# eezkni/UEGAN

Measured on AMD Instinct MI355X. Metric: train imgs/sec @512px bs=16 on 1/2/4/8 MI355X; infer ms/img, higher is better.
Workload: dtype bf16; 1 GPU; FiveK-shaped 512x512 batch=16/GPU, full G/D/VGG train step (trainer.py:77-119), conv_dim=32, seeded stand-in VGG19; global_batch=16, parallelism=dp1, pool_size=50, collective=none (1 rank), passes=batched (fused.py)

## Files before the change

### include/uegan_hip.h

```cpp
#ifndef UEGAN_HIP_H_
#define UEGAN_HIP_H_

#include <stddef.h>
#include <stdint.h>

#ifdef __cplusplus
extern "C" {
#endif

#define UEGAN_VERSION 105

enum { UEGAN_OK = 0, UEGAN_E_INVALID = -1, UEGAN_E_HIP = -2, UEGAN_E_UNSUPPORTED = -3 };
enum { UEGAN_F32 = 0, UEGAN_BF16 = 1 };
enum { UEGAN_PAD_ZERO = 0, UEGAN_PAD_REFLECT = 1 };
enum { UEGAN_ACT_NONE = 0, UEGAN_ACT_LRELU = 1, UEGAN_ACT_RELU = 2, UEGAN_ACT_TANH = 3,
       UEGAN_ACT_SIGMOID = 4,
       UEGAN_ACT_SWISH = 5, UEGAN_ACT_SELU = 6 };
enum { UEGAN_IMPL_AUTO = 0, UEGAN_IMPL_MFMA = 1, UEGAN_IMPL_DIRECT = 2, UEGAN_IMPL_MFMA_REGSTAGE = 3, UEGAN_IMPL_MFMA_GENERIC = 4 };

typedef void* uegan_stream_t;

int uegan_version(void);
const char* uegan_last_error(void);
int uegan_set_conv_impl(int impl);
enum {
  UEGAN_TUNE_SMALL_GRID = 0,
  UEGAN_TUNE_FOLD_MAX = 1,
  UEGAN_TUNE_HEADS_NO_CG = 2,
  UEGAN_TUNE_WIDE_MIN_GRID = 3,
  UEGAN_TUNE_TALL_MIN_GRID = 4,
  UEGAN_TUNE_TALL_RPW = 5,
  UEGAN_TUNE_TALL_REFLECT = 6,
  UEGAN_TUNE_FLAT_S2 = 7,
  UEGAN_TUNE_TOEP_HEADS = 8,
  UEGAN_TUNE_HEADS_MFMA = 9,
  UEGAN_TUNE_FWD_STATS = 10,
  UEGAN_TUNE_WGRAD_XCD = 11,
  UEGAN_TUNE_COUNT = 12
};
int uegan_set_tuning(int knob, int value, int* previous);
int uegan_selftest_mfma(void* scratch_4096_floats, uegan_stream_t stream);

typedef struct {
  char name[96];
  int64_t launches;
  double total_ms;
  double total_flops;
  double total_bytes;
} uegan_profile_entry;
int uegan_profile_begin(int max_records);
int uegan_profile_end(uegan_profile_entry* out, int max_entries, int* n_entries);

typedef struct {
// ... 71 lines not shown
int uegan_conv2d_fwd_pool_part(const uegan_conv_desc* d, const void* x1, const void* x2, const void* w_ohwi, const float* bias,
                               const float* scale, void* y, void* y_pool, int n_full, uegan_stream_t stream);
int uegan_conv2d_fwd_pool_idx(const uegan_conv_desc* d, const void* x1, const void* x2, const void* w_ohwi, const float* bias,
                              const float* scale, void* y, void* y_pool, void* idx, int n_full, int n_idx, uegan_stream_t stream);
int uegan_conv2d_dgrad(const uegan_conv_desc* d, const void* dz, const void* w_ihwo, const float* scale, void* dx1,
                       void* dx2, uegan_stream_t stream);
size_t uegan_conv2d_dgrad_workspace_bytes(const uegan_conv_desc* d);
int uegan_conv2d_dgrad_ws(const uegan_conv_desc* d, const void* dz, const void* w_ihwo, const float* scale, void* dx1,
                          void* dx2, void* workspace, size_t workspace_bytes, uegan_stream_t stream);
int uegan_conv2d_dgrad_padded(const uegan_conv_desc* d, const void* dz, const void* w_ihwo, const void* w_ohwi, const float* scale,
                              void* workspace, size_t workspace_bytes, int* pad_out, uegan_stream_t stream);
size_t uegan_conv2d_dgrad_padded_bytes(const uegan_conv_desc* d);

int uegan_conv2d_dgrad_act(const uegan_conv_desc* d, const void* dz, const void* w_ihwo, const float* scale, void* dx1,
                           void* workspace, size_t workspace_bytes, int in_act, const void* x_act, uegan_stream_t stream);
size_t uegan_conv2d_wgrad_workspace_bytes(const uegan_conv_desc* d);
int uegan_conv2d_wgrad(const uegan_conv_desc* d, const void* x1, const void* x2, const void* dz, const float* scale,
                       float* dw_oihw, float* dbias, void* workspace, size_t workspace_bytes, uegan_stream_t stream);
int uegan_conv2d_wgrad_acc(const uegan_conv_desc* d, const void* x1, const void* x2, const void* dz, const float* scale,
                           float* dw_oihw, float* dbias, void* workspace, size_t workspace_bytes, int accumulate,
                           uegan_stream_t stream);
int uegan_act_bwd(int dtype, int act, const void* g, const void* a, void* dz, int64_t n, uegan_stream_t stream);
int uegan_act_bwd2(int dtype, int act, const void* g, const void* g2, const void* a, void* dz, int64_t n, uegan_stream_t stream);
int uegan_act_bwd3(int dtype, int act, const void* g, const void* g2, const void* g3, const void* a, void* dz, int64_t n,
                   uegan_stream_t stream);

int uegan_nchw_to_nhwc(int dtype, const float* x_nchw, void* y_nhwc, int B, int C, int Cp, int H, int W, const float* a,
                       const float* b, uegan_stream_t stream);
int uegan_nhwc_to_nchw(int dtype, const void* x_nhwc, float* y_nchw, int B, int C, int Cp, int H, int W, const float* a,
                       uegan_stream_t stream);
// ... 144 lines not shown
```

### uegan_amd/_lib.py

```python
import ctypes as C
import os

_HERE = os.path.dirname(os.path.abspath(__file__))
LIB_PATH = os.path.join(_HERE, "libuegan_hip.so")
LIB_PATH_F16 = os.path.join(_HERE, "libuegan_hip_f16.so")

_lib = None
_lib_f16 = None
_use_f16 = False
_emulated = False

c_int, c_i64, c_f32, c_vp, c_sz = C.c_int, C.c_int64, C.c_float, C.c_void_p, C.c_size_t


class ConvDesc(C.Structure):
    _fields_ = [(n, C.c_int32) for n in ("dtype", "B", "H", "W", "C1", "C2", "Ho", "Wo", "Cout", "KH", "KW", "stride", "pad",
                                          "pad_mode", "act", "Cin_w", "Cout_w", "Cin_total", "scale_group")]


class ProfileEntry(C.Structure):
    _fields_ = [("name", C.c_char * 96), ("launches", c_i64), ("total_ms", C.c_double), ("total_flops", C.c_double),
                ("total_bytes", C.c_double)]


# ... 35 lines not shown
    "uegan_conv2d_fwd_ex": (c_int, [C.POINTER(ConvDesc), C.POINTER(ConvEx), c_vp, c_vp, c_vp, c_vp, c_vp, c_vp, C.POINTER(c_int), c_vp]),
    "uegan_nchw_to_nhwc_pair": (c_int, [c_int, c_vp, c_vp, c_int, c_int, c_int, c_int, c_int, C.POINTER(c_f32), C.POINTER(c_f32), c_vp]),
    "uegan_instnorm_apply_pair": (c_int, [c_int, c_vp, c_vp, c_vp, c_vp, c_vp, c_vp, c_int, c_int, c_int, c_vp]),
    "uegan_conv2d_fwd": (c_int, [C.POINTER(ConvDesc), c_vp, c_vp, c_vp, c_vp, c_vp, c_vp, c_vp]),
    "uegan_conv2d_fwd_splitk_workspace_bytes": (c_sz, [C.POINTER(ConvDesc)]),
    "uegan_conv2d_fwd_splitk": (c_int, [C.POINTER(ConvDesc), c_vp, c_vp, c_vp, c_vp, c_vp, c_vp, c_vp, c_sz, c_vp]),
    "uegan_conv2d_fwd_pool": (c_int, [C.POINTER(ConvDesc), c_vp, c_vp, c_vp, c_vp, c_vp, c_vp, c_vp, c_vp]),
    "uegan_conv2d_fwd_pool_part": (c_int, [C.POINTER(ConvDesc), c_vp, c_vp, c_vp, c_vp, c_vp, c_vp, c_vp, c_int, c_vp]),
    "uegan_conv2d_fwd_pool_idx": (c_int, [C.POINTER(ConvDesc), c_vp, c_vp, c_vp, c_vp, c_vp, c_vp, c_vp, c_vp, c_int, c_int, c_vp]),
    "uegan_maxpool2x2_fwd_idx": (c_int, [c_int, c_vp, c_vp, c_vp, c_int, c_int, c_int, c_int, c_vp]),
    "uegan_maxpool2x2_bwd_idx": (c_int, [c_int, c_int, c_vp, c_vp, c_vp, c_vp, c_int, c_int, c_int, c_int, c_vp]),
    "uegan_conv2d_dgrad": (c_int, [C.POINTER(ConvDesc), c_vp, c_vp, c_vp, c_vp, c_vp, c_vp]),
    "uegan_conv2d_dgrad_workspace_bytes": (c_sz, [C.POINTER(ConvDesc)]),
    "uegan_conv2d_dgrad_ws": (c_int, [C.POINTER(ConvDesc), c_vp, c_vp, c_vp, c_vp, c_vp, c_vp, c_sz, c_vp]),
    "uegan_conv2d_dgrad_act": (c_int, [C.POINTER(ConvDesc), c_vp, c_vp, c_vp, c_vp, c_vp, c_sz, c_int, c_vp, c_vp]),
    "uegan_conv2d_fwd_stats_workspace_bytes": (c_sz, [C.POINTER(ConvDesc)]),
    "uegan_conv2d_fwd_stats": (c_int, [C.POINTER(ConvDesc), c_vp, c_vp, c_vp, c_vp, c_vp, c_vp, c_vp, c_vp, c_f32, c_vp, c_sz, C.POINTER(c_int), c_vp]),
    "uegan_instnorm_apply": (c_int, [c_int, c_vp, c_vp, c_vp, c_vp, c_int, c_int, c_int, c_vp]),
    "uegan_conv2d_dgrad_padded": (c_int, [C.POINTER(ConvDesc), c_vp, c_vp, c_vp, c_vp, c_vp, c_sz, C.POINTER(c_int), c_vp]),
    "uegan_conv2d_dgrad_padded_bytes": (c_sz, [C.POINTER(ConvDesc)]),
    "uegan_conv2d_wgrad_workspace_bytes": (c_sz, [C.POINTER(ConvDesc)]),
    "uegan_conv2d_wgrad": (c_int, [C.POINTER(ConvDesc), c_vp, c_vp, c_vp, c_vp, c_vp, c_vp, c_vp, c_sz, c_vp]),
    "uegan_conv2d_wgrad_acc": (c_int, [C.POINTER(ConvDesc), c_vp, c_vp, c_vp, c_vp, c_vp, c_vp, c_vp, c_sz, c_int, c_vp]),
    "uegan_act_bwd": (c_int, [c_int, c_int, c_vp, c_vp, c_vp, c_i64, c_vp]),
    "uegan_act_bwd2": (c_int, [c_int, c_int, c_vp, c_vp, c_vp, c_vp, c_i64, c_vp]),
    "uegan_act_bwd3": (c_int, [c_int, c_int, c_vp, c_vp, c_vp, c_vp, c_vp, c_i64, c_vp]),
    "uegan_nchw_to_nhwc": (c_int, [c_int, c_vp, c_vp, c_int, c_int, c_int, c_int, c_int, C.POINTER(c_f32), C.POINTER(c_f32), c_vp]),
    "uegan_nhwc_to_nchw": (c_int, [c_int, c_vp, c_vp, c_int, c_int, c_int, c_int, c_int, C.POINTER(c_f32), c_vp]),
    "uegan_residual_clamp_fwd": (c_int, [c_int, c_vp, c_vp, c_vp, c_int, c_int, c_int, c_int, c_int, c_vp]),
    "uegan_residual_clamp_bwd": (c_int, [c_int, c_vp, c_vp, c_vp, c_vp, c_vp, c_int, c_int, c_int, c_int, c_int, c_vp]),
# ... 141 lines not shown
```

### uegan_amd/csrc/common.h

```cpp
#pragma once
#include <hip/hip_runtime.h>
#include <stdint.h>
#include <stddef.h>

#include "../../include/uegan_hip.h"

#ifdef UEGAN_TOOLS_BUILD
#define UEGAN_ABL_BITS(x) (x)
#else
#define UEGAN_ABL_BITS(x) 0
#endif

namespace uegan {

extern int g_tuning[UEGAN_TUNE_COUNT];
extern int g_abl_stream, g_abl_wide;


typedef uint16_t bf16_t;

typedef float f32x4 __attribute__((ext_vector_type(4)));
typedef short s16x8 __attribute__((ext_vector_type(8)));
typedef uint32_t u32x4 __attribute__((ext_vector_type(4)));
typedef uint32_t u32x2 __attribute__((ext_vector_type(2)));
// ... 141 lines not shown
    default: return apply_act_ext(v, act);
  }
}
__device__ __forceinline__ float act_grad_of_pre(float v, int act) {
  switch (act) {
    case UEGAN_ACT_LRELU: return v > 0.f ? 1.f : 0.2f;
    case UEGAN_ACT_RELU: return v > 0.f ? 1.f : 0.f;
    case UEGAN_ACT_TANH: { const float t = tanhf(v); return 1.f - t * t; }
    case UEGAN_ACT_SIGMOID: { const float sg = 1.f / (1.f + expf(-v)); return sg * (1.f - sg); }
    case UEGAN_ACT_SWISH: { const float sg = 1.f / (1.f + expf(-v)); return sg * (1.f + v * (1.f - sg)); }
    case UEGAN_ACT_SELU: return v > 0.f ? UEGAN_SELU_SCALE : (UEGAN_SELU_SCALE * UEGAN_SELU_ALPHA) * expf(v);
    default: return 1.f;
  }
}

__host__ __device__ __forceinline__ int reflect_idx(int i, int n) {
  i = i < 0 ? -i : i;
  return i >= n ? 2 * (n - 1) - i : i;
}

__device__ __forceinline__ float wave_sum(float v) {
#pragma unroll
  for (int o = 32; o > 0; o >>= 1) v += __shfl_xor(v, o, 64);
  return v;
}

__device__ __forceinline__ float block_sum(float v, float* red) {
  v = wave_sum(v);
  const int lane = threadIdx.x & 63, w = threadIdx.x >> 6;
  __syncthreads();
// ... 35 lines not shown
```

### uegan_amd/csrc/conv.hip

```cpp
#include "conv_core.h"

#include <type_traits>

namespace uegan {

static int g_conv_impl = UEGAN_IMPL_AUTO;
int g_tuning[UEGAN_TUNE_COUNT] = {256, -1, 0, 192, 192, 0, 1, 1, 1, 1, 1, 1};
int g_abl_stream = 0, g_abl_wide = 0;
#ifdef UEGAN_TOOLS_BUILD
extern "C" int uegan_tools_set_ablation(int stream_wgrad_bits, int wide_variant) {
  g_abl_stream = stream_wgrad_bits;
  g_abl_wide = wide_variant;
  return UEGAN_OK;
}
#endif

bool g_prof_on = false;
std::vector<ProfRecord> g_prof_records;
std::vector<std::pair<hipEvent_t, hipEvent_t>> g_prof_pool;
size_t g_prof_used = 0;

int conv_patch_bf16_a(ConvArgs& a, hipStream_t s, int ks);
int conv_patch_bf16_b(ConvArgs& a, hipStream_t s, int ks);
int conv_patch_f32_a(ConvArgs& a, hipStream_t s, int ks);
// ... 1709 lines not shown
    g.B = d->B; g.IH = d->Ho; g.IW = d->Wo; g.C1 = d->Cout; g.C2 = 0; g.C = d->Cout;
    g.OH = d->H; g.OW = d->W; g.KH = d->KH; g.KW = d->KW; g.stride = d->stride; g.pad = d->pad; g.pad_mode = d->pad_mode;
    g.mode = 1;
    a.in1 = dz; a.in2 = dz; a.bias = nullptr; a.nbias = 0; a.scale = scale; a.scale_group = d->scale_group; a.act = UEGAN_ACT_NONE;
    a.Kp = (int)uegan_packed_k((int64_t)d->KH * d->KW * d->Cout);
    a.w = w_ihwo; a.N = d->C1;
    a.out = dx1; a.out2 = nullptr; a.n_out1 = d->C1;
    a.frame = 0; a.fy0 = a.fy1 = a.fx0 = a.fx1 = 0; a.mask = nullptr; a.mask_act = UEGAN_ACT_NONE;
    a.mask = x_act; a.mask_act = in_act;
    rc = d->dtype == UEGAN_F32 ? run_gather_gemm<float>(a, s, &applied) : run_gather_gemm<bf16_t>(a, s, &applied);
  }
  if (rc || applied) return rc;
  return uegan_act_bwd(d->dtype, in_act, dx1, x_act, dx1, (int64_t)d->B * d->H * d->W * d->C1, stream);
}

static void wgrad_plan(const uegan_conv_desc* d, WgradArgs& a, int& nsplit, dim3& grid, int& bn, WgradTrPlan& tr) {
  a.g = fwd_geom(d);
  a.N = cout_w(d);
  a.zC = d->Cout;
  a.ktot = d->KH * d->KW * (d->C1 + d->C2);
  if (g_conv_impl != UEGAN_IMPL_DIRECT && wgtr_plan(d, a.g, tr)) {
    bn = -1;
    nsplit = tr.nsplit_eff;
    grid = tr.grid;
    return;
  }
  const int npix = d->dtype == UEGAN_BF16 ? 64 : 32;
  int ws = 1, wl = 0;
  while (ws < d->Wo && ws < npix) { ws <<= 1; ++wl; }
  a.WS = ws; a.WSlog = wl; a.R = npix / ws;
// ... 280 lines not shown
```

### uegan_amd/csrc/conv_core.h

```cpp
#pragma once
#include "common.h"
#include "conv_internal.h"

#include <stdio.h>
#include <stdlib.h>
#include <utility>
#include <vector>

namespace uegan {

struct ProfRecord {
  hipEvent_t start, stop;
  int kernel_id;
  double flops, bytes;
};
extern bool g_prof_on;
extern std::vector<ProfRecord> g_prof_records;
extern std::vector<std::pair<hipEvent_t, hipEvent_t>> g_prof_pool;
extern size_t g_prof_used;

static inline int prof_key(int kind, bool bf16, int bn, int ks, int mode, int th, bool glds) {
  return (kind << 28) | ((bf16 ? 1 : 0) << 24) | (bn << 12) | (ks << 8) | (mode << 4) | ((th == 32 ? 2 : (th == 16 ? 1 : (th == 4 ? 3 : 0))) << 1) | (glds ? 1 : 0);
}
static void prof_kernel_name(int key, char* buf, size_t n) {
// ... 170 lines not shown
  void* out;
  void* out2;
  int n_out1;
  int N, Kp, act, nbias;
  int nty, ntx;
  int frame;
  int fy0, fy1, fx0, fx1;
  const void* mask;
  int mask_act;
  void* pool_out = nullptr;
  int pool_done = 0;
  void* pool_idx = nullptr;
  int n_idx = 0;
  int n_full = 1 << 30;
  int xcd_map = 0;
  int rect_y0 = 0, rect_y1 = 0, rect_x0 = 0, rect_x1 = 0;
  int border_only = 0;
  float* stats_part = nullptr;
  int stats_tpi = 0;
  const void* in1_lo = nullptr;
  const void* in2_lo = nullptr;
  const void* w_lo = nullptr;
  void* out_lo = nullptr;
  const void* mul = nullptr;
  const void* mul_lo = nullptr;
  void* out_mul = nullptr;
  void* out_mul_lo = nullptr;
  int src_wrap = 0;
  const float* res_x = nullptr;
  const float* res_x2 = nullptr;
// ... 28 lines not shown
```

### uegan_amd/csrc/conv_internal.h

```cpp
#pragma once
#include <hip/hip_runtime.h>

#include "../../include/uegan_hip.h"

namespace uegan {
bool heads_applicable(const uegan_conv_desc* d);
int heads_fwd(const uegan_conv_desc* d, const void* x, const void* w_ohwi, const float* bias, const float* scale, void* y, hipStream_t s);
bool heads_dgrad_applicable(const uegan_conv_desc* d);
int heads_dgrad(const uegan_conv_desc* d, const void* dz, const void* w_ihwo, const float* scale, void* dx, hipStream_t s);
int heads_wgrad_blocks(const uegan_conv_desc* d);
int heads_wgrad(const uegan_conv_desc* d, const void* x, const void* dz, float* ws, hipStream_t s);
}
```

### uegan_amd/csrc/conv_wide.hip

```cpp
#include "conv_core.h"

namespace uegan {

static __device__ __attribute__((aligned(128))) const unsigned int g_zero_page[512] = {0u};

typedef float f32x16 __attribute__((ext_vector_type(16)));

__device__ __forceinline__ f32x16 mfma32_bf16(u32x4 a, u32x4 b, f32x16 c) {
#ifdef UEGAN_HALF_FP16
  return __builtin_amdgcn_mfma_f32_32x32x16_f16(__builtin_bit_cast(bf16x8_t, a), __builtin_bit_cast(bf16x8_t, b), c, 0, 0, 0);
#else
  return __builtin_amdgcn_mfma_f32_32x32x16_bf16(__builtin_bit_cast(bf16x8_t, a), __builtin_bit_cast(bf16x8_t, b), c, 0, 0, 0);
#endif
}

#define UEGAN_SB() __builtin_amdgcn_sched_barrier(0)

template <int KS, int MODE, bool MASK, int ABL = 0>
__global__ void __launch_bounds__(256, 1) conv_wide_kernel(ConvArgs a) {
  constexpr int TH = 8, TW = 32, BN = 256, NWAVES = 4;
  constexpr int PH = TH + KS - 1, PW = TW + KS - 1;
  constexpr int NPG = (PH * PW + 7) / 8;
  constexpr int NI_P = (NPG + NWAVES - 1) / NWAVES;
  constexpr int PBUFB = NPG * 1024, WHALF = BN * 64, DUMPB = 4096;
// ... 238 lines not shown
      if (MASK) {
        const u32x4 m = *reinterpret_cast<const u32x4*>(static_cast<const bf16_t*>(a.mask) + o);
#pragma unroll
        for (int d = 0; d < 4; ++d) {
          const float lo = half_lo_to_f32(v[d]) * (half_lo_to_f32(m[d]) > 0.f ? 1.f : mslope);
          const float hi = half_hi_to_f32(v[d]) * (half_hi_to_f32(m[d]) > 0.f ? 1.f : mslope);
          v[d] = pack_bf16x2(lo, hi);
        }
      }
      bf16_t* dst = !a.out2 ? out + o : (nl < a.n_out1 ? out + pix * a.n_out1 + nl : static_cast<bf16_t*>(a.out2) + pix * (a.N - a.n_out1) + (nl - a.n_out1));
      *reinterpret_cast<u32x4*>(dst) = v;
    }
  }
}

template <int NI, int MODE, bool MASK, bool POOL, int RPW = 4>
__global__ void __launch_bounds__(256, RPW == 2 ? 2 : 1) conv_tall_kernel(ConvArgs a) {
  static_assert(RPW == 4 || RPW == 2, "rows per wave");
  constexpr bool REFL = MODE == 2;
  static_assert(!REFL || (NI == 4 && !MASK && !POOL), "mirrored images: 128-channel blocks, plain epilogue");
  constexpr int KS = 3, TH = 4 * RPW, TW = 32, BN = NI * 32, NWAVES = 4;
  constexpr int PH = TH + KS - 1, PW = TW + KS - 1, NPIX = PH * PW;
  constexpr int NPG = (NPIX + 15) / 16;
  constexpr int NI_P = (NPG + NWAVES - 1) / NWAVES;
  constexpr int PBUFB = NPG * 1024, WSL = BN * 64, NWP = WSL / 1024 / NWAVES;
  constexpr int DUMPB = RPW == 2 ? 1024 : 4096, DUMPW = RPW == 2 ? 0 : 1024;
  constexpr int NT = KS * KS, NLOAD = NWP + 2;
  constexpr bool DGRAD = MODE != 0;
  constexpr int EROW = BN * 2 + 8;
  constexpr int WPIX = RPW * 32;
  constexpr int MAINB = 2 * PBUFB + 4 * WSL, EPIB = NWAVES * WPIX * EROW;
  constexpr int BODYB = MAINB > EPIB ? MAINB : EPIB;
  static_assert(NI_P <= 2 * (NT - 2), "the next chunk's patch pieces must be requested two steps before the chunk ends");
  static_assert((RPW == 2 ? 2 : 1) * (BODYB + DUMPB + BN * 4) <= 160 * 1024, "LDS budget");
  static_assert(NWP >= 1, "at least one weight piece per wave per slice");
// ... 249 lines not shown
        MF(wf1, xf1, 0, 3) LDX(xf0, pnext, 0, 2) LDX(xf0, pnext, 0, 3) UEGAN_SB();
        MF(wf1, xf1, 1, 0) MF(wf1, xf1, 1, 1) MF(wf1, xf1, 1, 2) MF(wf1, xf1, 1, 3)
      }
      if (RPW == 2 && NI == 2 && 2 * tap >= NI_P) wait_vmcnt<NWP>();
      else wait_vmcnt<NLOAD>();
      raw_barrier();
    }
  }
#undef MF
#undef LDW
#undef LDX
#undef FOLDX
  wait_vmcnt<0>();

  unsigned char* const est = lds + wave * (WPIX * EROW);
  {
    const float slope = a.act == UEGAN_ACT_LRELU ? 0.2f : (a.act == UEGAN_ACT_RELU ? 0.f : 1.f);
#pragma unroll
    for (int i = 0; i < NI; ++i) {
      f32x4 bv[4];
#pragma unroll
      for (int q = 0; q < 4; ++q) bv[q] = *reinterpret_cast<const f32x4*>(lds_bias + (i * 32 + 4 * lh + 8 * q) * 4);
#pragma unroll
      for (int j = 0; j < RPW; ++j) {
        unsigned char* row = est + (j * 32 + l31) * EROW + i * 64 + 8 * lh;
#pragma unroll
        for (int q = 0; q < 4; ++q) {
          float v[4];
#pragma unroll
          for (int r = 0; r < 4; ++r) {
// ... 4 lines not shown
          pk.x = pack_bf16x2(v[0], v[1]);
          pk.y = pack_bf16x2(v[2], v[3]);
          *reinterpret_cast<u32x2*>(row + q * 16) = pk;
        }
      }
    }
  }
  __builtin_amdgcn_wave_barrier();
  {
    constexpr int LPP = BN / 8;
    constexpr int PPI = 64 / LPP;
    const float mslope = a.mask_act == UEGAN_ACT_LRELU ? 0.2f : (a.mask_act == UEGAN_ACT_RELU ? 0.f : 1.f);
    bf16_t* out = static_cast<bf16_t*>(a.out);
    const int lc = lane % LPP, nl = n0 + lc * 8;
    const int n_store = (POOL && b >= a.n_full) ? 0 : WPIX / PPI;
#pragma unroll 4
    for (int it = 0; it < n_store; ++it) {
      const int rr = it * PPI + lane / LPP;
      const int oy = y0 + wave * RPW + (rr >> 5), ox = x0 + (rr & 31);
      const u32x2 v01 = *reinterpret_cast<const u32x2*>(est + rr * EROW + lc * 16);
      const u32x2 v23 = *reinterpret_cast<const u32x2*>(est + rr * EROW + lc * 16 + 8);
      u32x4 v = {v01.x, v01.y, v23.x, v23.y};
      if (oy >= g.OH || ox >= g.OW) continue;
      const size_t pix = ((size_t)b * g.OH + oy) * g.OW + ox;
      const size_t o = pix * a.N + nl;
      if (MASK) {
        const u32x4 m = *reinterpret_cast<const u32x4*>(static_cast<const bf16_t*>(a.mask) + o);
#pragma unroll
        for (int d = 0; d < 4; ++d) {
          const float lo = half_lo_to_f32(v[d]) * (half_lo_to_f32(m[d]) > 0.f ? 1.f : mslope);
          const float hi = half_hi_to_f32(v[d]) * (half_hi_to_f32(m[d]) > 0.f ? 1.f : mslope);
          v[d] = pack_bf16x2(lo, hi);
        }
      }
      bf16_t* dst = !a.out2 ? out + o : (nl < a.n_out1 ? out + pix * a.n_out1 + nl : static_cast<bf16_t*>(a.out2) + pix * (a.N - a.n_out1) + (nl - a.n_out1));
      *reinterpret_cast<u32x4*>(dst) = v;
    }
    if constexpr (POOL) {
      bf16_t* pout = static_cast<bf16_t*>(a.pool_out);
      const int PH2 = g.OH >> 1, PW2 = g.OW >> 1;
#pragma unroll 2
      for (int it = 0; it < WPIX / 4 / PPI; ++it) {
        const int pp = it * PPI + lane / LPP;
        const int pr = pp >> 4, pc = pp & 15;
        const int py = ((y0 + wave * RPW) >> 1) + pr, px = (x0 >> 1) + pc;
        float m[8];
        uint32_t arg[8];
#pragma unroll
// ... 26 lines not shown
  }
}

int conv_tall_run(ConvArgs& a, int dtype, hipStream_t s, bool interior) {
  const ConvGeom& g = a.g;
  const int min_grid = g_tuning[UEGAN_TUNE_TALL_MIN_GRID];
  if (min_grid < 0) return 1;
  if (dtype != UEGAN_BF16 || g.stride != 1 || g.KH != 3 || g.KW != 3 || a.frame != 0) return 1;
  if (g.C1 % 32 || g.C2 % 32 || g.C > 1024 || (a.N != 64 && a.N % 128) || g.OW < 32 || g.OH < 16) return 1;
  const bool refl = !interior && g.mode == 1 && g.pad_mode == UEGAN_PAD_REFLECT && g.pad == 1 && !g.C2 && !a.mask && a.N % 128 == 0 &&
                    (!a.out2 || a.n_out1 % 8 == 0) && g.OH >= 4 && g.OW >= 4 && g_tuning[UEGAN_TUNE_TALL_REFLECT] != 0;
  if (!interior && !refl && (a.out2 || (g.mode == 1 && (g.C2 || (g.pad_mode == UEGAN_PAD_REFLECT && g.pad != 0))))) return 1;
  if (interior && (g.mode != 1 || g.C2 || a.mask || (a.out2 && a.n_out1 % 8))) return 1;
  auto simple = [](int act) { return act == UEGAN_ACT_NONE || act == UEGAN_ACT_LRELU || act == UEGAN_ACT_RELU; };
  if (!simple(a.act) || (a.mask && !simple(a.mask_act))) return 1;
  const int rpw_knob = g_tuning[UEGAN_TUNE_TALL_RPW];
  bool rpw2 = rpw_knob == 2 || (rpw_knob != 4 && g.C < 512);
  const int nb_n = a.N == 64 ? 1 : a.N / 128;
  {
    const int ntx = interior ? (a.rect_x1 - a.rect_x0) / 32 : (g.OW + 31) / 32;
    const int nty16 = interior ? (a.rect_y1 - a.rect_y0) / 16 : (g.OH + 15) / 16, nty8 = interior ? (a.rect_y1 - a.rect_y0) / 8 : (g.OH + 7) / 8;
    if (g.B * nty16 * ntx * nb_n < min_grid) {
      if (rpw_knob == 4 || g.B * nty8 * ntx * nb_n < min_grid) return 1;
      rpw2 = true;
    }
  }
  const int th = rpw2 ? 8 : 16;
  a.nty = interior ? (a.rect_y1 - a.rect_y0) / th : (g.OH + th - 1) / th;
  a.ntx = interior ? (a.rect_x1 - a.rect_x0) / 32 : (g.OW + 31) / 32;
  const int gm = g.B * a.nty * a.ntx;
  const bool pool = a.pool_out && g.mode == 0 && !a.mask && g.OH % 2 == 0 && g.OW % 2 == 0;
  const double rows = interior ? (double)g.B * (a.rect_y1 - a.rect_y0) * (a.rect_x1 - a.rect_x0) : (g.mode == 0 ? (double)g.B * g.OH * g.OW : (double)g.B * g.IH * g.IW);
  ProfScope prof(prof_key(7, true, a.N == 64 ? 64 : 128, 3, refl ? 2 : g.mode, 16, !pool), 2.0 * rows * a.N * (double)(9 * g.C), s,
                 2.0 * (rows * a.N + (interior ? rows : (double)g.B * g.IH * g.IW) * g.C));
  const dim3 grid(gm, a.N == 64 ? 1 : a.N / 128), block(256);
  a.xcd_map = (grid.y > 1 && gm % 8 == 0) ? 1 : 0;
#define UEGAN_TALL(NI, RPW)                                                                                          \
  do {                                                                                                               \
    if (g.mode == 0 && pool) hipLaunchKernelGGL((conv_tall_kernel<NI, 0, false, true, RPW>), grid, block, 0, s, a);  \
    else if (g.mode == 0) hipLaunchKernelGGL((conv_tall_kernel<NI, 0, false, false, RPW>), grid, block, 0, s, a);    \
    else if (a.mask) hipLaunchKernelGGL((conv_tall_kernel<NI, 1, true, false, RPW>), grid, block, 0, s, a);          \
    else hipLaunchKernelGGL((conv_tall_kernel<NI, 1, false, false, RPW>), grid, block, 0, s, a);                     \
  } while (0)
  if (refl) {
    if (rpw2) hipLaunchKernelGGL((conv_tall_kernel<4, 2, false, false, 2>), grid, block, 0, s, a);
    else hipLaunchKernelGGL((conv_tall_kernel<4, 2, false, false, 4>), grid, block, 0, s, a);
  }
  else if (a.N == 64) { if (rpw2) UEGAN_TALL(2, 2); else UEGAN_TALL(2, 4); }
  else if (rpw2) UEGAN_TALL(4, 2);
  else UEGAN_TALL(4, 4);
#undef UEGAN_TALL
  if (g.mode == 0 && pool) a.pool_done = 1;
  UEGAN_CHECK_LAUNCH();
  return UEGAN_OK;
}
// ... 52 lines not shown
```

### uegan_amd/csrc/norm_loss.hip

```cpp
#include "common.h"

namespace uegan {

struct RedPlan {
  int B, HW, C;
  int V;
  int CG;
  int PL;
  int ncg;
  int S;
  int chunk;
};

static RedPlan make_plan(int B, int HW, int C, int epc) {
  RedPlan p;
  p.B = B; p.HW = HW; p.C = C;
  p.V = (C % epc == 0) ? epc : 1;
  const int lanes = C / p.V;
  int cg = 1;
  while (cg < lanes && cg < 64) cg <<= 1;
  p.CG = cg;
  p.PL = 256 / cg;
  p.ncg = (lanes + cg - 1) / cg;
  int s = (HW + 1023) / 1024;
// ... 359 lines not shown
__global__ void percep_loss_kernel(const float* tot, float weight, float* loss, RedPlan p) {
  __shared__ float red[16];
  const int total = p.B * p.C;
  float acc = 0.f;
  for (int i = blockIdx.x * blockDim.x + threadIdx.x; i < total; i += gridDim.x * blockDim.x) acc += tot[(size_t)i * 3];
  acc = block_sum(acc, red);
  const float nel = (float)p.B * (float)p.HW * (float)p.C;
  if (threadIdx.x == 0) *loss += weight * acc / nel;
}

template <typename T, int V, bool RELU, bool ACC = false>
__global__ void percep_grad_kernel(const T* x, const T* y, const float* st, const float* tot, float weight, const float* gscale, T* gx,
                                   RedPlan p, int act) {
  RED_THREAD_SETUP();
  if (!cvalid) return;
  const float nel = (float)p.B * (float)p.HW * (float)p.C;
  const float k = 2.f * weight * (gscale ? *gscale : 1.f) / nel, inv_n = 1.f / (float)p.HW;
  const size_t bc = (size_t)p.B * p.C, o0 = (size_t)b * p.C + c0;
  float mx[V], rx[V], my[V], ry[V], mg[V], mgx[V];
#pragma unroll
  for (int e = 0; e < V; ++e) {
    mx[e] = st[o0 + e]; rx[e] = st[bc + o0 + e]; my[e] = st[2 * bc + o0 + e]; ry[e] = st[3 * bc + o0 + e];
    mg[e] = k * tot[(o0 + e) * 3 + 1] * inv_n;
    mgx[e] = k * tot[(o0 + e) * 3 + 2] * inv_n;
  }
  _Pragma("unroll 4") for (int q = p0 + pl; q < p1; q += p.PL) {
    float xv[V], yv[V];
    Vec<T, V>::ld(x + base + (size_t)q * p.C, xv);
    Vec<T, V>::ld(y + base + (size_t)q * p.C, yv);
#pragma unroll
    for (int e = 0; e < V; ++e) {
      const float xh = (xv[e] - mx[e]) * rx[e], yh = (yv[e] - my[e]) * ry[e];
      const float gv = rx[e] * (k * (xh - yh) - mg[e] - xh * mgx[e]);
      xv[e] = RELU ? (xv[e] > 0.f ? gv : 0.f) : gv * act_grad_from_out(xv[e], act);
    }
    if (ACC) {
      float pv[V];
      Vec<T, V>::ld(gx + base + (size_t)q * p.C, pv);
#pragma unroll
      for (int e = 0; e < V; ++e) xv[e] += pv[e];
    }
    Vec<T, V>::st(gx + base + (size_t)q * p.C, xv);
  }
}

constexpr int RB = 64;
__device__ __forceinline__ float fold_partials(const float* part, int nb) {
  const int lane = threadIdx.x & 63;
// ... 585 lines not shown
                                          const float* ca, const float* cb, const float* cc, void* gx, int B, int HW, int C, uegan_stream_t stream) {
  UEGAN_CHECK_ARG(gy && x && gx && B > 0 && HW > 0 && C > 0 && act >= UEGAN_ACT_NONE && act <= UEGAN_ACT_SELU, "bad affine_act args");
  RedPlan p = make_plan(B, HW, C, epc_of(dtype));
  DISPATCH_TV(dtype, p.V, hipLaunchKernelGGL((affine_act_bwd_apply_kernel<T, V>), dim3(p.S, p.ncg, B), dim3(256), 0, (hipStream_t)stream,
                                             (const T*)gy, (const T*)x, scale, shift, act, ca, cb, cc, (T*)gx, p));
  UEGAN_CHECK_LAUNCH();
  return UEGAN_OK;
}

static void percep_layout(const RedPlan& p, float* tmp, float*& px, float*& py, float*& sums, float*& st, float*& tot) {
  const size_t part = (size_t)p.B * p.S * p.C * 3, region = part + (size_t)p.B * p.C * 8;
  px = tmp; py = tmp + region; sums = tmp + 2 * region;
  st = tmp + part;
  tot = tmp + 2 * region + part;
}

extern "C" int uegan_percep_tap_fwd(int dtype, const void* x, const void* y, float weight, float* loss, float* tmp, int B, int HW, int C,
                                    float eps, uegan_stream_t stream) {
  UEGAN_CHECK_ARG(x && y && loss && tmp && B > 0 && HW > 0 && C > 0, "bad percep args");
  RedPlan p = make_plan(B, HW, C, epc_of(dtype));
  dim3 grid(p.S, p.ncg, B);
  hipStream_t s = (hipStream_t)stream;
  float *px, *py, *sums, *st, *tot;
  percep_layout(p, tmp, px, py, sums, st, tot);
  const size_t bc = (size_t)B * C;
  DISPATCH_TV(dtype, p.V, hipLaunchKernelGGL((moments_partial_kernel<T, V>), grid, dim3(256), 0, s, (const T*)x, px, p));
  UEGAN_CHECK_LAUNCH();
  DISPATCH_TV(dtype, p.V, hipLaunchKernelGGL((moments_partial_kernel<T, V>), grid, dim3(256), 0, s, (const T*)y, py, p));
  UEGAN_CHECK_LAUNCH();
  hipLaunchKernelGGL(moments_finalize_kernel, dim3(bc_blocks(p, 1)), dim3(256), 0, s, px, st, st + bc, p, eps);
// ... 335 lines not shown
```

### uegan_amd/fused.py

```python
import ctypes as C

import torch

from . import _lib as L
from . import ops
from .ops import ACT_NONE, ACT_RELU, _dt, _p, _stream, lib


class _VGGFidelityFn(torch.autograd.Function):

    @staticmethod
    def forward(ctx, x, y, vgg, weights, a, b, y_taps=None):
        from .losses import VGG_TAP_IDX
        B = x.shape[0]
        need = ctx.needs_input_grad[0]
        dt = ops.get_compute_dtype()
        h = ops.raw_to_nhwc([x, y] if y_taps is None else [x], dt, a, b)
        st = _stream()
        recs, taps, tap_stats = [], [], []
        pooled = None
        pool_idx = None
        for pi, (kind, idx) in enumerate(vgg.plan):
            if kind == "pool":
                Bt, H, W, Cc = h.shape
# ... 40 lines not shown
                L.check(lib().uegan_percep_tap_fwd(_dt(t), _p(t), _p(ty), float(w), _p(loss), _p(tmp), B, H * W, Cc, ops.IN_EPS, st))
            tmps.append(tmp)
        if need:
            ctx.recs, ctx.taps, ctx.tmps, ctx.weights, ctx.a, ctx.B, ctx.C = recs, taps, tmps, weights, a, B, x.shape[1]
            ctx.ytaps = y_taps
            ctx.last = h
        return loss.reshape(())

    @staticmethod
    def backward(ctx, g):
        B = ctx.B
        g = g.contiguous().float().reshape(1)
        st = _stream()
        cur = None
        ti = len(ctx.taps) - 1
        for li in range(len(ctx.recs) - 1, -1, -1):
            kind, xin, d, ihwo, is_tap = ctx.recs[li]
            if kind == "pool":
                yp, pidx, (Bt, H, W, Cc) = d
                gx = torch.empty((B, H, W, Cc), dtype=yp.dtype, device=yp.device)
                if pidx is not None:
                    L.check(lib().uegan_maxpool2x2_bwd_idx(_dt(yp), ACT_RELU, _p(yp), _p(pidx), _p(cur), _p(gx), B, H, W, Cc, st))
                else:
                    L.check(lib().uegan_maxpool2x2_bwd_act(_dt(xin), ACT_RELU, _p(xin), _p(cur), _p(gx), B, H, W, Cc, st))
                cur = gx
                continue
            if is_tap:
                t, tmp, w = ctx.taps[ti], ctx.tmps[ti], ctx.weights[ti]
                ti -= 1
                _, H, W, Cc = t.shape
                acc = 1
                if cur is None:
                    cur = torch.empty((B, H, W, Cc), dtype=t.dtype, device=t.device)
                    acc = 0
                ty = t[B:] if ctx.ytaps is None else ctx.ytaps[ti + 1]
                L.check(lib().uegan_percep_tap_bwd_acc(_dt(t), ACT_RELU, _p(t), _p(ty), float(w), _p(g), _p(cur), _p(tmp), B, H * W, Cc,
                                                       ops.IN_EPS, acc, st))
            if cur is None:
                continue
            if li == 0:
                dx, _ = ops.raw_conv_dgrad(d, cur, ihwo, nb=B)
                return ops.raw_to_nchw_grad(dx, ctx.C, ctx.a), None, None, None, None, None, None
            prev_is_conv = ctx.recs[li - 1][0] == "conv"
            cur, _ = ops.raw_conv_dgrad(d, cur, ihwo, in_act=ACT_RELU if prev_is_conv else ACT_NONE, x_act=xin if prev_is_conv else None, nb=B)
        raise RuntimeError("VGG plan does not start with a convolution")


def vgg_fidelity_loss(vgg, weights, x, y, a, b, y_taps=None):
    if not vgg.deferred_act_grad:
        raise RuntimeError("the fused fidelity loss applies every ReLU gradient at the consumers (VGG19_relu(deferred_act_grad=True))")
    return _VGGFidelityFn.apply(x, y, vgg, tuple(weights), a, b, None if y_taps is None else tuple(y_taps))


@torch.no_grad()
def vgg_reference_taps(vgg, y, a, b):
    from .losses import VGG_TAP_IDX
    h = ops.raw_to_nhwc([y], ops.get_compute_dtype(), a, b)
    st = _stream()
    taps, pooled = [], None
    for pi, (kind, idx) in enumerate(vgg.plan):
# ... 208 lines not shown
```

Measured before the change: 496.5 imgs/sec.

## Fuse perceptual-tap gradient and max-unpool into VGG dgrad tall-kernel epilogue

Adds two epilogue variants to the tall conv dgrad kernel used in the VGG fidelity-loss backward. One adds the perceptual-tap instance-norm gradient (with ReLU mask) directly into the dgrad output. The other scatters the dgrad result through the saved max-pool indices into the full-resolution gradient. This removes the separate tap-backward and maxpool-backward kernels and their extra reads and writes of large activations. In exchange the epilogue does more register and memory work, and it falls back to the old path when the tall kernel is not eligible.

```diff
diff --git a/include/uegan_hip.h b/include/uegan_hip.h
--- a/include/uegan_hip.h
+++ b/include/uegan_hip.h
@@ -36,7 +36,8 @@
   UEGAN_TUNE_HEADS_MFMA = 9,
   UEGAN_TUNE_FWD_STATS = 10,
   UEGAN_TUNE_WGRAD_XCD = 11,
-  UEGAN_TUNE_COUNT = 12
+  UEGAN_TUNE_VGG_EPI = 12,
+  UEGAN_TUNE_COUNT = 13
 };
 int uegan_set_tuning(int knob, int value, int* previous);
 int uegan_selftest_mfma(void* scratch_4096_floats, uegan_stream_t stream);
@@ -138,6 +139,11 @@
 
 int uegan_conv2d_dgrad_act(const uegan_conv_desc* d, const void* dz, const void* w_ihwo, const float* scale, void* dx1,
                            void* workspace, size_t workspace_bytes, int in_act, const void* x_act, uegan_stream_t stream);
+int uegan_conv2d_dgrad_act_tap(const uegan_conv_desc* d, const void* dz, const void* w_ihwo, const float* scale, void* dx1, int in_act,
+                               const void* x_act, const void* y, float weight, const float* gscale, const float* tmp, int* applied,
+                               uegan_stream_t stream);
+int uegan_conv2d_dgrad_unpool(const uegan_conv_desc* d, const void* dz, const void* w_ihwo, const float* scale, void* dx_full, int in_act,
+                              const void* y_pool, const void* idx, int* applied, uegan_stream_t stream);
 size_t uegan_conv2d_wgrad_workspace_bytes(const uegan_conv_desc* d);
 int uegan_conv2d_wgrad(const uegan_conv_desc* d, const void* x1, const void* x2, const void* dz, const float* scale,
                        float* dw_oihw, float* dbias, void* workspace, size_t workspace_bytes, uegan_stream_t stream);
diff --git a/uegan_amd/_lib.py b/uegan_amd/_lib.py
--- a/uegan_amd/_lib.py
+++ b/uegan_amd/_lib.py
@@ -73,6 +73,8 @@
     "uegan_conv2d_dgrad_workspace_bytes": (c_sz, [C.POINTER(ConvDesc)]),
     "uegan_conv2d_dgrad_ws": (c_int, [C.POINTER(ConvDesc), c_vp, c_vp, c_vp, c_vp, c_vp, c_vp, c_sz, c_vp]),
     "uegan_conv2d_dgrad_act": (c_int, [C.POINTER(ConvDesc), c_vp, c_vp, c_vp, c_vp, c_vp, c_sz, c_int, c_vp, c_vp]),
+    "uegan_conv2d_dgrad_act_tap": (c_int, [C.POINTER(ConvDesc), c_vp, c_vp, c_vp, c_vp, c_int, c_vp, c_vp, c_f32, c_vp, c_vp, C.POINTER(c_int), c_vp]),
+    "uegan_conv2d_dgrad_unpool": (c_int, [C.POINTER(ConvDesc), c_vp, c_vp, c_vp, c_vp, c_int, c_vp, c_vp, C.POINTER(c_int), c_vp]),
     "uegan_conv2d_fwd_stats_workspace_bytes": (c_sz, [C.POINTER(ConvDesc)]),
     "uegan_conv2d_fwd_stats": (c_int, [C.POINTER(ConvDesc), c_vp, c_vp, c_vp, c_vp, c_vp, c_vp, c_vp, c_vp, c_f32, c_vp, c_sz, C.POINTER(c_int), c_vp]),
     "uegan_instnorm_apply": (c_int, [c_int, c_vp, c_vp, c_vp, c_vp, c_int, c_int, c_int, c_vp]),
diff --git a/uegan_amd/csrc/common.h b/uegan_amd/csrc/common.h
--- a/uegan_amd/csrc/common.h
+++ b/uegan_amd/csrc/common.h
@@ -179,6 +179,22 @@
   }
 }
 
+__device__ __forceinline__ void percep_scalars(float weight, const float* gscale, int B, int HW, int C, float& k, float& inv_n) {
+  const float nel = (float)B * (float)HW * (float)C;
+  k = 2.f * weight * (gscale ? *gscale : 1.f) / nel;
+  inv_n = 1.f / (float)HW;
+}
+__device__ __forceinline__ void percep_consts(const float* st, const float* tot, size_t bc, size_t o, float k, float inv_n, float& mx, float& rx,
+                                              float& my, float& ry, float& mg, float& mgx) {
+  mx = st[o]; rx = st[bc + o]; my = st[2 * bc + o]; ry = st[3 * bc + o];
+  mg = k * tot[o * 3 + 1] * inv_n;
+  mgx = k * tot[o * 3 + 2] * inv_n;
+}
+__device__ __forceinline__ float percep_tap_grad(float x, float y, float mx, float rx, float my, float ry, float k, float mg, float mgx) {
+  const float xh = (x - mx) * rx, yh = (y - my) * ry;
+  return rx * (k * (xh - yh) - mg - xh * mgx);
+}
+
 __host__ __device__ __forceinline__ int reflect_idx(int i, int n) {
   i = i < 0 ? -i : i;
   return i >= n ? 2 * (n - 1) - i : i;
diff --git a/uegan_amd/csrc/conv.hip b/uegan_amd/csrc/conv.hip
--- a/uegan_amd/csrc/conv.hip
+++ b/uegan_amd/csrc/conv.hip
@@ -5,7 +5,7 @@
 namespace uegan {
 
 static int g_conv_impl = UEGAN_IMPL_AUTO;
-int g_tuning[UEGAN_TUNE_COUNT] = {256, -1, 0, 192, 192, 0, 1, 1, 1, 1, 1, 1};
+int g_tuning[UEGAN_TUNE_COUNT] = {256, -1, 0, 192, 192, 0, 1, 1, 1, 1, 1, 1, 1};
 int g_abl_stream = 0, g_abl_wide = 0;
 #ifdef UEGAN_TOOLS_BUILD
 extern "C" int uegan_tools_set_ablation(int stream_wgrad_bits, int wide_variant) {
@@ -1747,6 +1747,65 @@
   return uegan_act_bwd(d->dtype, in_act, dx1, x_act, dx1, (int64_t)d->B * d->H * d->W * d->C1, stream);
 }
 
+static void dgrad_epi_args(const uegan_conv_desc* d, const void* dz, const void* w_ihwo, const float* scale, void* out, ConvArgs& a) {
+  ConvGeom& g = a.g;
+  g.B = d->B; g.IH = d->Ho; g.IW = d->Wo; g.C1 = d->Cout; g.C2 = 0; g.C = d->Cout;
+  g.OH = d->H; g.OW = d->W; g.KH = d->KH; g.KW = d->KW; g.stride = d->stride; g.pad = d->pad; g.pad_mode = d->pad_mode;
+  g.mode = 1;
+  a.in1 = dz; a.in2 = dz; a.bias = nullptr; a.nbias = 0; a.scale = scale; a.scale_group = d->scale_group; a.act = UEGAN_ACT_NONE;
+  a.Kp = (int)uegan_packed_k((int64_t)d->KH * d->KW * d->Cout);
+  a.w = w_ihwo; a.N = d->C1;
+  a.out = out; a.out2 = nullptr; a.n_out1 = d->C1;
+  a.frame = 0; a.fy0 = a.fy1 = a.fx0 = a.fx1 = 0; a.mask = nullptr; a.mask_act = UEGAN_ACT_NONE;
+}
+static bool dgrad_takes_tall(const uegan_conv_desc* d, const ConvArgs& a) {
+  const ConvGeom& g = a.g;
+  if (d->dtype != UEGAN_BF16 || d->C2 || g_conv_impl == UEGAN_IMPL_DIRECT || !g_use_glds || !g_use_patch || g_tuning[UEGAN_TUNE_VGG_EPI] == 0) return false;
+  if (dgrad_folds(d) || (g_use_heads && heads_dgrad_applicable(d))) return false;
+  if (g_use_stream && conv_toep_takes(a, d->dtype)) return false;
+  ConvStreamPlan sp;
+  if (conv_stream_plan(a, d->dtype, sp)) return false;
+  return g.stride == 1 && g.KH == 3 && g.KW == 3 && g.pad_mode != UEGAN_PAD_REFLECT && g.C % (CONV_ROWB / 2) == 0;
+}
+
+extern "C" int uegan_conv2d_dgrad_act_tap(const uegan_conv_desc* d, const void* dz, const void* w_ihwo, const float* scale, void* dx1, int in_act,
+                                          const void* x_act, const void* y, float weight, const float* gscale, const float* tmp, int* applied,
+                                          uegan_stream_t stream) {
+  int rc = check_desc(d);
+  if (rc) return rc;
+  UEGAN_CHECK_ARG(dz && w_ihwo && dx1 && x_act && y && tmp && applied, "null pointer");
+  *applied = 0;
+  ConvArgs a;
+  dgrad_epi_args(d, dz, w_ihwo, scale, dx1, a);
+  a.mask = x_act; a.mask_act = in_act;
+  if (in_act != UEGAN_ACT_RELU || !dgrad_takes_tall(d, a)) return UEGAN_OK;
+  a.epi = 1;
+  a.epi_y = y; a.epi_weight = weight; a.epi_gscale = gscale;
+  percep_tap_consts(d->dtype, tmp, d->B, d->H * d->W, d->C1, &a.epi_st, &a.epi_tot);
+  rc = conv_tall_run(a, d->dtype, (hipStream_t)stream);
+  if (rc == 1) return UEGAN_OK;
+  if (rc == UEGAN_OK) *applied = 1;
+  return rc;
+}
+
+extern "C" int uegan_conv2d_dgrad_unpool(const uegan_conv_desc* d, const void* dz, const void* w_ihwo, const float* scale, void* dx_full, int in_act,
+                                         const void* y_pool, const void* idx, int* applied, uegan_stream_t stream) {
+  int rc = check_desc(d);
+  if (rc) return rc;
+  UEGAN_CHECK_ARG(dz && w_ihwo && dx_full && y_pool && idx && applied, "null pointer");
+  *applied = 0;
+  ConvArgs a;
+  dgrad_epi_args(d, dz, w_ihwo, scale, dx_full, a);
+  if (in_act != UEGAN_ACT_RELU || !dgrad_takes_tall(d, a)) return UEGAN_OK;
+  a.mask = y_pool; a.mask_act = in_act;
+  a.epi = 2;
+  a.epi_idx = static_cast<const unsigned char*>(idx);
+  rc = conv_tall_run(a, d->dtype, (hipStream_t)stream);
+  if (rc == 1) return UEGAN_OK;
+  if (rc == UEGAN_OK) *applied = 1;
+  return rc;
+}
+
 static void wgrad_plan(const uegan_conv_desc* d, WgradArgs& a, int& nsplit, dim3& grid, int& bn, WgradTrPlan& tr) {
   a.g = fwd_geom(d);
   a.N = cout_w(d);
diff --git a/uegan_amd/csrc/conv_core.h b/uegan_amd/csrc/conv_core.h
--- a/uegan_amd/csrc/conv_core.h
+++ b/uegan_amd/csrc/conv_core.h
@@ -208,6 +208,13 @@
   int n_idx = 0;
   int n_full = 1 << 30;
   int xcd_map = 0;
+  int epi = 0;
+  const void* epi_y = nullptr;
+  const float* epi_st = nullptr;
+  const float* epi_tot = nullptr;
+  const float* epi_gscale = nullptr;
+  float epi_weight = 0.f;
+  const unsigned char* epi_idx = nullptr;
   int rect_y0 = 0, rect_y1 = 0, rect_x0 = 0, rect_x1 = 0;
   int border_only = 0;
   float* stats_part = nullptr;
diff --git a/uegan_amd/csrc/conv_internal.h b/uegan_amd/csrc/conv_internal.h
--- a/uegan_amd/csrc/conv_internal.h
+++ b/uegan_amd/csrc/conv_internal.h
@@ -10,4 +10,5 @@
 int heads_dgrad(const uegan_conv_desc* d, const void* dz, const void* w_ihwo, const float* scale, void* dx, hipStream_t s);
 int heads_wgrad_blocks(const uegan_conv_desc* d);
 int heads_wgrad(const uegan_conv_desc* d, const void* x, const void* dz, float* ws, hipStream_t s);
+void percep_tap_consts(int dtype, const float* tmp, int B, int HW, int C, const float** st, const float** tot);
 }
diff --git a/uegan_amd/csrc/conv_wide.hip b/uegan_amd/csrc/conv_wide.hip
--- a/uegan_amd/csrc/conv_wide.hip
+++ b/uegan_amd/csrc/conv_wide.hip
@@ -276,11 +276,12 @@
   }
 }
 
-template <int NI, int MODE, bool MASK, bool POOL, int RPW = 4>
+template <int NI, int MODE, bool MASK, bool POOL, int RPW = 4, int EPI = 0>
 __global__ void __launch_bounds__(256, RPW == 2 ? 2 : 1) conv_tall_kernel(ConvArgs a) {
   static_assert(RPW == 4 || RPW == 2, "rows per wave");
   constexpr bool REFL = MODE == 2;
   static_assert(!REFL || (NI == 4 && !MASK && !POOL), "mirrored images: 128-channel blocks, plain epilogue");
+  static_assert(EPI == 0 || (MODE == 1 && MASK && !POOL), "fidelity-loss epilogues: masked data gradients");
   constexpr int KS = 3, TH = 4 * RPW, TW = 32, BN = NI * 32, NWAVES = 4;
   constexpr int PH = TH + KS - 1, PW = TW + KS - 1, NPIX = PH * PW;
   constexpr int NPG = (NPIX + 15) / 16;
@@ -560,6 +561,23 @@
   wait_vmcnt<0>();
 
   unsigned char* const est = lds + wave * (WPIX * EROW);
+  float tst[EPI == 1 ? 32 : 1], ttot[EPI == 1 ? 24 : 1], tgs = 1.f;
+  if constexpr (EPI == 1) {
+    const size_t bc = (size_t)g.B * a.N, o0 = (size_t)b * a.N + n0 + (lane % (BN / 8)) * 8;
+#pragma unroll
+    for (int q = 0; q < 8; ++q) {
+      const f32x4 v = *reinterpret_cast<const f32x4*>(a.epi_st + (q >> 1) * bc + o0 + 4 * (q & 1));
+#pragma unroll
+      for (int e = 0; e < 4; ++e) tst[4 * q + e] = v[e];
+    }
+#pragma unroll
+    for (int q = 0; q < 6; ++q) {
+      const f32x4 v = *reinterpret_cast<const f32x4*>(a.epi_tot + o0 * 3 + 4 * q);
+#pragma unroll
+      for (int e = 0; e < 4; ++e) ttot[4 * q + e] = v[e];
+    }
+    if (a.epi_gscale) tgs = *a.epi_gscale;
+  }
   {
     const float slope = a.act == UEGAN_ACT_LRELU ? 0.2f : (a.act == UEGAN_ACT_RELU ? 0.f : 1.f);
 #pragma unroll
@@ -594,6 +612,14 @@
     bf16_t* out = static_cast<bf16_t*>(a.out);
     const int lc = lane % LPP, nl = n0 + lc * 8;
     const int n_store = (POOL && b >= a.n_full) ? 0 : WPIX / PPI;
+    float tmx[EPI == 1 ? 8 : 1], trx[EPI == 1 ? 8 : 1], tmy[EPI == 1 ? 8 : 1], try_[EPI == 1 ? 8 : 1], tmg[EPI == 1 ? 8 : 1], tmgx[EPI == 1 ? 8 : 1];
+    float tk = 0.f;
+    if constexpr (EPI == 1) {
+      float inv_n;
+      percep_scalars(a.epi_weight, &tgs, g.B, g.OH * g.OW, a.N, tk, inv_n);
+#pragma unroll
+      for (int e = 0; e < 8; ++e) percep_consts(tst, ttot, 8, e, tk, inv_n, tmx[e], trx[e], tmy[e], try_[e], tmg[e], tmgx[e]);
+    }
 #pragma unroll 4
     for (int it = 0; it < n_store; ++it) {
       const int rr = it * PPI + lane / LPP;
@@ -606,12 +632,38 @@
       const size_t o = pix * a.N + nl;
       if (MASK) {
         const u32x4 m = *reinterpret_cast<const u32x4*>(static_cast<const bf16_t*>(a.mask) + o);
+        u32x4 yv = {0u, 0u, 0u, 0u};
+        if constexpr (EPI == 1) yv = *reinterpret_cast<const u32x4*>(static_cast<const bf16_t*>(a.epi_y) + o);
 #pragma unroll
         for (int d = 0; d < 4; ++d) {
-          const float lo = half_lo_to_f32(v[d]) * (half_lo_to_f32(m[d]) > 0.f ? 1.f : mslope);
-          const float hi = half_hi_to_f32(v[d]) * (half_hi_to_f32(m[d]) > 0.f ? 1.f : mslope);
+          float lo = half_lo_to_f32(v[d]) * (half_lo_to_f32(m[d]) > 0.f ? 1.f : mslope);
+          float hi = half_hi_to_f32(v[d]) * (half_hi_to_f32(m[d]) > 0.f ? 1.f : mslope);
+          if constexpr (EPI == 1) {
+            const float xl = half_lo_to_f32(m[d]), xh = half_hi_to_f32(m[d]);
+            const float gl = percep_tap_grad(xl, half_lo_to_f32(yv[d]), tmx[2 * d], trx[2 * d], tmy[2 * d], try_[2 * d], tk, tmg[2 * d], tmgx[2 * d]);
+            const float gh = percep_tap_grad(xh, half_hi_to_f32(yv[d]), tmx[2 * d + 1], trx[2 * d + 1], tmy[2 * d + 1], try_[2 * d + 1], tk,
+                                             tmg[2 * d + 1], tmgx[2 * d + 1]);
+            lo = (xl > 0.f ? gl : 0.f) + lo;
+            hi = (xh > 0.f ? gh : 0.f) + hi;
+          }
           v[d] = pack_bf16x2(lo, hi);
         }
+      }
+      if constexpr (EPI == 2) {
+        const u32x2 a8 = *reinterpret_cast<const u32x2*>(a.epi_idx + o);
+        const size_t ow2 = 2 * (size_t)g.OW;
+        bf16_t* base = out + (((size_t)b * 2 * g.OH + 2 * oy) * ow2 + 2 * ox) * a.N + nl;
+#pragma unroll
+        for (int k = 0; k < 4; ++k) {
+          u32x4 w4;
+#pragma unroll
+          for (int d = 0; d < 4; ++d) {
+            const uint32_t by = a8[d >> 1] >> (16 * (d & 1));
+            w4[d] = v[d] & (((by & 0xffu) == (uint32_t)k ? 0xffffu : 0u) | (((by >> 8) & 0xffu) == (uint32_t)k ? 0xffff0000u : 0u));
+          }
+          *reinterpret_cast<u32x4*>(base + ((k >> 1) * ow2 + (k & 1)) * a.N) = w4;
+        }
+        continue;
       }
       bf16_t* dst = !a.out2 ? out + o : (nl < a.n_out1 ? out + pix * a.n_out1 + nl : static_cast<bf16_t*>(a.out2) + pix * (a.N - a.n_out1) + (nl - a.n_out1));
       *reinterpret_cast<u32x4*>(dst) = v;
@@ -668,6 +720,7 @@
   if (interior && (g.mode != 1 || g.C2 || a.mask || (a.out2 && a.n_out1 % 8))) return 1;
   auto simple = [](int act) { return act == UEGAN_ACT_NONE || act == UEGAN_ACT_LRELU || act == UEGAN_ACT_RELU; };
   if (!simple(a.act) || (a.mask && !simple(a.mask_act))) return 1;
+  if (a.epi && (interior || refl || g.mode != 1 || !a.mask || a.mask_act != UEGAN_ACT_RELU || a.out2 || g.C2)) return 1;
   const int rpw_knob = g_tuning[UEGAN_TUNE_TALL_RPW];
   bool rpw2 = rpw_knob == 2 || (rpw_knob != 4 && g.C < 512);
   const int nb_n = a.N == 64 ? 1 : a.N / 128;
@@ -693,6 +746,8 @@
   do {                                                                                                               \
     if (g.mode == 0 && pool) hipLaunchKernelGGL((conv_tall_kernel<NI, 0, false, true, RPW>), grid, block, 0, s, a);  \
     else if (g.mode == 0) hipLaunchKernelGGL((conv_tall_kernel<NI, 0, false, false, RPW>), grid, block, 0, s, a);    \
+    else if (a.mask && a.epi == 1) hipLaunchKernelGGL((conv_tall_kernel<NI, 1, true, false, RPW, 1>), grid, block, 0, s, a); \
+    else if (a.mask && a.epi == 2) hipLaunchKernelGGL((conv_tall_kernel<NI, 1, true, false, RPW, 2>), grid, block, 0, s, a); \
     else if (a.mask) hipLaunchKernelGGL((conv_tall_kernel<NI, 1, true, false, RPW>), grid, block, 0, s, a);          \
     else hipLaunchKernelGGL((conv_tall_kernel<NI, 1, false, false, RPW>), grid, block, 0, s, a);                     \
   } while (0)
diff --git a/uegan_amd/csrc/norm_loss.hip b/uegan_amd/csrc/norm_loss.hip
--- a/uegan_amd/csrc/norm_loss.hip
+++ b/uegan_amd/csrc/norm_loss.hip
@@ -1,4 +1,5 @@
 #include "common.h"
+#include "conv_internal.h"
 
 namespace uegan {
 
@@ -397,24 +398,19 @@
                                    RedPlan p, int act) {
   RED_THREAD_SETUP();
   if (!cvalid) return;
-  const float nel = (float)p.B * (float)p.HW * (float)p.C;
-  const float k = 2.f * weight * (gscale ? *gscale : 1.f) / nel, inv_n = 1.f / (float)p.HW;
+  float k, inv_n;
+  percep_scalars(weight, gscale, p.B, p.HW, p.C, k, inv_n);
   const size_t bc = (size_t)p.B * p.C, o0 = (size_t)b * p.C + c0;
   float mx[V], rx[V], my[V], ry[V], mg[V], mgx[V];
 #pragma unroll
-  for (int e = 0; e < V; ++e) {
-    mx[e] = st[o0 + e]; rx[e] = st[bc + o0 + e]; my[e] = st[2 * bc + o0 + e]; ry[e] = st[3 * bc + o0 + e];
-    mg[e] = k * tot[(o0 + e) * 3 + 1] * inv_n;
-    mgx[e] = k * tot[(o0 + e) * 3 + 2] * inv_n;
-  }
+  for (int e = 0; e < V; ++e) percep_consts(st, tot, bc, o0 + e, k, inv_n, mx[e], rx[e], my[e], ry[e], mg[e], mgx[e]);
   _Pragma("unroll 4") for (int q = p0 + pl; q < p1; q += p.PL) {
     float xv[V], yv[V];
     Vec<T, V>::ld(x + base + (size_t)q * p.C, xv);
     Vec<T, V>::ld(y + base + (size_t)q * p.C, yv);
 #pragma unroll
     for (int e = 0; e < V; ++e) {
-      const float xh = (xv[e] - mx[e]) * rx[e], yh = (yv[e] - my[e]) * ry[e];
-      const float gv = rx[e] * (k * (xh - yh) - mg[e] - xh * mgx[e]);
+      const float gv = percep_tap_grad(xv[e], yv[e], mx[e], rx[e], my[e], ry[e], k, mg[e], mgx[e]);
       xv[e] = RELU ? (xv[e] > 0.f ? gv : 0.f) : gv * act_grad_from_out(xv[e], act);
     }
     if (ACC) {
@@ -1030,6 +1026,13 @@
   st = tmp + part;
   tot = tmp + 2 * region + part;
 }
+void uegan::percep_tap_consts(int dtype, const float* tmp, int B, int HW, int C, const float** st, const float** tot) {
+  RedPlan p = make_plan(B, HW, C, epc_of(dtype));
+  float *px, *py, *sums, *s, *t;
+  percep_layout(p, const_cast<float*>(tmp), px, py, sums, s, t);
+  *st = s;
+  *tot = t;
+}
 
 extern "C" int uegan_percep_tap_fwd(int dtype, const void* x, const void* y, float weight, float* loss, float* tmp, int B, int HW, int C,
                                     float eps, uegan_stream_t stream) {
diff --git a/uegan_amd/fused.py b/uegan_amd/fused.py
--- a/uegan_amd/fused.py
+++ b/uegan_amd/fused.py
@@ -78,9 +78,12 @@
         st = _stream()
         cur = None
         ti = len(ctx.taps) - 1
+        folded = set()
         for li in range(len(ctx.recs) - 1, -1, -1):
             kind, xin, d, ihwo, is_tap = ctx.recs[li]
             if kind == "pool":
+                if li in folded:
+                    continue
                 yp, pidx, (Bt, H, W, Cc) = d
                 gx = torch.empty((B, H, W, Cc), dtype=yp.dtype, device=yp.device)
                 if pidx is not None:
@@ -89,7 +92,9 @@
                     L.check(lib().uegan_maxpool2x2_bwd_act(_dt(xin), ACT_RELU, _p(xin), _p(cur), _p(gx), B, H, W, Cc, st))
                 cur = gx
                 continue
-            if is_tap:
+            if is_tap and li in folded:
+                ti -= 1
+            elif is_tap:
                 t, tmp, w = ctx.taps[ti], ctx.tmps[ti], ctx.weights[ti]
                 ti -= 1
                 _, H, W, Cc = t.shape
@@ -105,9 +110,41 @@
             if li == 0:
                 dx, _ = ops.raw_conv_dgrad(d, cur, ihwo, nb=B)
                 return ops.raw_to_nchw_grad(dx, ctx.C, ctx.a), None, None, None, None, None, None
-            prev_is_conv = ctx.recs[li - 1][0] == "conv"
+            prev = ctx.recs[li - 1]
+            prev_is_conv = prev[0] == "conv"
+            if prev_is_conv and prev[4]:
+                ty = ctx.taps[ti][B:] if ctx.ytaps is None else ctx.ytaps[ti]
+                dx = _dgrad_tap(d, cur, ihwo, xin, ty, ctx.weights[ti], g, ctx.tmps[ti], B)
+                if dx is not None:
+                    cur = dx
+                    folded.add(li - 1)
+                    continue
+            elif not prev_is_conv and prev[2][1] is not None:
+                yp, pidx, (Bt, H, W, Cc) = prev[2]
+                gx = _dgrad_unpool(d, cur, ihwo, yp, pidx, (B, H, W, Cc), B)
+                if gx is not None:
+                    cur = gx
+                    folded.add(li - 1)
+                    continue
             cur, _ = ops.raw_conv_dgrad(d, cur, ihwo, in_act=ACT_RELU if prev_is_conv else ACT_NONE, x_act=xin if prev_is_conv else None, nb=B)
         raise RuntimeError("VGG plan does not start with a convolution")
+
+
+def _dgrad_tap(d, dz, ihwo, t, ty, w, g, tmp, nb):
+    d = ops._sub_desc(d, nb)
+    dx = torch.empty((d.B, d.H, d.W, d.C1), dtype=dz.dtype, device=dz.device)
+    ok = C.c_int(0)
+    L.check(lib().uegan_conv2d_dgrad_act_tap(C.byref(d), _p(dz), _p(ihwo), None, _p(dx), ACT_RELU, _p(t), _p(ty), float(w), _p(g), _p(tmp),
+                                             C.byref(ok), _stream()))
+    return dx if ok.value else None
+
+
+def _dgrad_unpool(d, dz, ihwo, yp, pidx, full_shape, nb):
+    d = ops._sub_desc(d, nb)
+    gx = torch.empty(full_shape, dtype=dz.dtype, device=dz.device)
+    ok = C.c_int(0)
+    L.check(lib().uegan_conv2d_dgrad_unpool(C.byref(d), _p(dz), _p(ihwo), None, _p(gx), ACT_RELU, _p(yp), _p(pidx), C.byref(ok), _stream()))
+    return gx if ok.value else None
 
 
 def vgg_fidelity_loss(vgg, weights, x, y, a, b, y_taps=None):
```

Measured after the change: 504.9 imgs/sec (median of 6 runs). 1.02x the previous value.
